# brockpat/JKMP22-Machine-Learning-and-the-Implementable-Efficient-Frontier-Replication

Measured on AMD Instinct MI355X. Metric: PFML hp×window solves/sec (whole node); full grid-search wall-clock, S&P500, higher is better.
Workload: dtype fp64; 1 GPU; global_batch=42824, seq_len=710, parallelism=dp1, dist_backend=none, device=AMD Radeon Graphics, outputs_finite=True, includes_s4_inputs=False, ridge_solve_dtype=fp64 (lambda = 0 / rank-deficient systems: bf16 cannot carry them, SURVEY 7.4), hip_graph=True

## Files before the change

### jkmp22-machine-learning-and-the-implementable-efficient-frontier-replication_amd/csrc/ridge_band.hip

```cpp
#include "common.h"
#include "ridge_desc.h"
#include <cstdlib>
#include <type_traits>

namespace {

constexpr int BB = 16;
constexpr int LS = BB + 1;
constexpr int BMP = 512;
constexpr int BNMAX = BMP + BB;
constexpr int NTR = 512;
constexpr int NWR = NTR / 64;
constexpr int TBR = 4;
constexpr int NTB = 512;
constexpr int NWB = NTB / 64;
constexpr int LC = 16;

__host__ __device__ __forceinline__ int band_npad(int n) { return (n + BB - 1) & ~(BB - 1); }

struct BandWork {
  double *A, *LB, *z, *T, *Yt, *Lf, *F;
  __device__ BandWork(double* w, int n, int L) {
    const int np = (n + BB - 1) / BB;
    const int npad = band_npad(n);
// ... 874 lines not shown
  auto stage_rows = [&](int r0s, int buf) {
    for (int e = threadIdx.x; e < BB * LS; e += NTS) {
      const int r = r0s + e / LS, s = e % LS;
      LBs[buf][e / LS][s] = (r < n) ? LB[(int64_t)r * LS + s] : (s == BB ? 1.0 : 0.0);
    }
  };
  static_assert(BB * LS <= 2 * NTS, "two staged doubles per thread");
  double st[2];
  auto load_rows = [&](int r0s) {
#pragma unroll
    for (int h = 0; h < 2; ++h) {
      const int e = threadIdx.x + h * NTS;
      const int r = r0s + e / LS, s = e % LS;
      st[h] = (e < BB * LS && r < n) ? LB[(int64_t)r * LS + s] : (s == BB ? 1.0 : 0.0);
    }
  };
  auto store_rows = [&](int buf) {
#pragma unroll
    for (int h = 0; h < 2; ++h) {
      const int e = threadIdx.x + h * NTS;
      if (e < BB * LS) LBs[buf][e / LS][e % LS] = st[h];
    }
  };
#pragma unroll
  for (int k = 0; k < 2 * BB; ++k)
    w[k] = (k <= p && p < n) ? LB[(int64_t)p * LS + BB - p + k] + (k == p ? lam : 0.0)
                             : (k == p ? 1.0 : 0.0);
  double zr = (p < n) ? z[p] : 0.0;
  stage_rows(BB, 0);
  double znx = (p + BB < n) ? z[p + BB] : 0.0;
  bool ok = true;
  __syncthreads();

  __builtin_amdgcn_s_waitcnt(0x0F70);
  auto fwd_block = [&](int j0, auto CHECK) {
    constexpr bool chk = decltype(CHECK)::value;
    const int sb = (j0 >> 4) & 1;
    const double lam_in = (j0 + BB + p < n) ? lam : 0.0;
    load_rows(j0 + 2 * BB);
    const double znx2 = (j0 + 2 * BB + p < n) ? z[j0 + 2 * BB + p] : 0.0;
    double myinv = 0.0, myy = 0.0;
    static_for<0, 16>([&](auto U) {
      constexpr int u = decltype(U)::value;
      const int j = j0 + u;
      const bool pl = (p == u);
      double piv = row_bcast<u>(w[u]);
      const double zpiv = row_bcast<u>(zr);
      lds_row_issue<u>(w, lbs_base + (unsigned)(sb * BB * LS + u * LS) * 8u, piv);
      ok = ok && (piv > 0.0);
      double inv = rsqrt1_f64(piv);
      lds_row_wait<u>(w, inv);
      const double yj = zpiv * inv;
      if (pl) {
        w[u + BB] += lam_in;
        zr = znx;
        myinv = inv;
        myy = yj;
      }
      const double lval = w[u] * inv;
      if (!chk || j < n) Lrow[(int64_t)j * BB + (pl ? BB - 1 : ((p - u) & 15) - 1)] = lval;
      zr -= lval * yj;
      static_for<1, LS>([&](auto K) {
        constexpr int k = decltype(K)::value;
        fnmac_bcast<(u + k) & 15, k == 1>(w[u + k], lval, lval);
      });
    });
    if (!chk || j0 + p < n) {
      Linv[j0 + p] = myinv;
      yl[j0 + p] = myy;
    }
#pragma unroll
    for (int s = 0; s < BB; ++s) w[s] = w[s + BB];
    znx = znx2;
    store_rows(sb ^ 1);
    __syncthreads();
  };
  for (int j0 = 0; j0 < npad - 16; j0 += 16) fwd_block(j0, std::false_type{});
  fwd_block(npad - 16, std::true_type{});
  __syncthreads();
  const long long t_mid = (long long)__builtin_amdgcn_s_memtime();
  struct Half {
    double pl[8], iv[8], yv[8];
  };
  auto load_half = [&](int jb, auto S0, auto CHECK, Half& h) {
    constexpr int s0 = decltype(S0)::value;
    static_for<0, 8>([&](auto V) {
      constexpr int v = decltype(V)::value;
      constexpr int u = 15 - s0 - v;
      const int j = jb - s0 - v;
      const int i = (p - u) & 15;
      if constexpr (decltype(CHECK)::value) {
        const bool in = j < n;
        h.pl[v] = in ? Lrow[(int64_t)j * BB + (i == 0 ? BB - 1 : i - 1)] : 0.0;
        h.iv[v] = in ? Linv[j] : 1.0;
        h.yv[v] = in ? yl[j] : 0.0;
      } else {
        const int jc = max(j, 0);
        h.pl[v] = Lrow[(int64_t)jc * BB + (i == 0 ? BB - 1 : i - 1)];
        h.iv[v] = Linv[jc];
        h.yv[v] = yl[jc];
      }
    });
  };
  double xr = 0.0, x1 = 0.0, x2 = 0.0;
  double Pq[2] = {0.0, 0.0}, L1q[2] = {0.0, 0.0}, L2q[2] = {0.0, 0.0};
  auto prep = [&](auto UP, double pl) {
    constexpr int up = decltype(UP)::value & 15;
    const int i = (p - up) & 15;
    const double pm = (i == 1 || i == 2) ? 0.0 : pl;
    Pq[0] = Pq[1];
    L1q[0] = L1q[1];
    L2q[0] = L2q[1];
    Pq[1] = row16_sum(pm * xr);
    L1q[1] = row_bcast<(up + 1) & 15>(pl);
    L2q[1] = row_bcast<(up + 2) & 15>(pl);
  };
  auto step = [&](double yv, double iv) {
    const double t = fma(-L2q[0], x2, yv - Pq[0]);
    const double xj = fma(-L1q[0], x1, t) * iv;
    x2 = x1;
    x1 = xj;
    return xj;
  };
  auto store_half = [&](int jb, int s0) {
    const int j = jb - (15 - p);
    if (lv && j < n && 15 - p >= s0 && 15 - p < s0 + 8) yl[j] = ok ? xr : __builtin_nan("");
  };
  using I0 = std::integral_constant<int, 0>;
  using I8 = std::integral_constant<int, 8>;
  Half A, B;
  load_half(npad - 1, I0{}, std::true_type{}, A);
  {
    Pq[1] = 0.0;
    L1q[1] = row_bcast<0>(A.pl[0]);
    L2q[1] = row_bcast<1>(A.pl[0]);
    Pq[0] = Pq[1]; L1q[0] = L1q[1]; L2q[0] = L2q[1];
    Pq[1] = 0.0;
    L1q[1] = row_bcast<15>(A.pl[1]);
    L2q[1] = row_bcast<0>(A.pl[1]);
  }
  auto block = [&](int jb, auto FIRST) {
    load_half(jb, I8{}, FIRST, B);
    static_for<0, 8>([&](auto V) {
      constexpr int v = decltype(V)::value;
      constexpr int u = 15 - v;
      const double xj = step(A.yv[v], A.iv[v]);
      if constexpr (v + 2 < 8) prep(std::integral_constant<int, u - 2>{}, A.pl[v + 2]);
      else prep(std::integral_constant<int, u - 2>{}, B.pl[v - 6]);
      xr = (p == u) ? xj : xr;
    });
    store_half(jb, 0);
    load_half(jb - 16, I0{}, std::false_type{}, A);
    static_for<0, 8>([&](auto V) {
      constexpr int v = decltype(V)::value;
      constexpr int u = 7 - v;
      const double xj = step(B.yv[v], B.iv[v]);
      if constexpr (v + 2 < 8) prep(std::integral_constant<int, u - 2 + 16>{}, B.pl[v + 2]);
      else prep(std::integral_constant<int, u - 2 + 16>{}, A.pl[v - 6]);
      xr = (p == u) ? xj : xr;
    });
    store_half(jb, 8);
  };
  block(npad - 1, std::true_type{});
  for (int jb = npad - 17; jb >= 0; jb -= 16) block(jb, std::false_type{});
  if (tim != nullptr && blockIdx.x == 0 && threadIdx.x == 0) {
    const long long t_end = (long long)__builtin_amdgcn_s_memtime();
    tim[(int64_t)ncells * 8 + 0] = t_mid - t_start;
    tim[(int64_t)ncells * 8 + 1] = t_end - t_mid;
  }
}

constexpr int LR = BB + 1;
constexpr int UW = 2 * BB + 1;
constexpr int LU_WG = 128;

__global__ __launch_bounds__(256) void band_lu_flag_kernel(const RidgeCellDesc* __restrict__ cells,
                                                           int ncells, int L,
                                                           double* __restrict__ work,
                                                           int* __restrict__ list,
                                                           int* __restrict__ count, int cap) {
  const int e = blockIdx.x * blockDim.x + threadIdx.x;
  if (e >= ncells * L) return;
  const int c = e / L, l = e % L;
  const RidgeCellDesc cd = cells[c];
  const BandWork bw(work + cd.work, cd.n, L);
  const double y0 = bw.Yt[(int64_t)l * cd.n];
  if (y0 != y0) {
    const int slot = atomicAdd(count, 1);
    if (slot < cap) list[slot] = e;
  }
}

__global__ __launch_bounds__(64) void ridge_band_lu_kernel(
    const RidgeCellDesc* __restrict__ cells, const double* __restrict__ lvec, int L,
    double* __restrict__ work, const int* __restrict__ list, const int* __restrict__ count,
    int cap) {
  __shared__ double Us[BNMAX][UW];
  __shared__ double ys[BNMAX];
  __shared__ double W[LR][UW];
  __shared__ double Z[LR];
  const int total = min(*count, cap);
  const int lane = threadIdx.x;
  for (int q = blockIdx.x; q < total; q += gridDim.x) {
    const int e = list[q];
    const RidgeCellDesc cd = cells[e / L];
    const int l = e % L, n = cd.n;
    BandWork bw(work + cd.work, n, L);
    const double lam = lvec[l];
    const double* __restrict__ LB = bw.LB;
    auto band = [&](int r, int c) -> double {
      if (r >= n || c >= n || c < 0 || abs(r - c) > BB) return 0.0;
      const int hi = max(r, c), lo = min(r, c);
      return LB[(int64_t)hi * LS + lo - hi + BB] + (r == c ? lam : 0.0);
    };
    for (int x = lane; x < LR * UW; x += 64) W[x / UW][x % UW] = band(x / UW, x % UW);
    if (lane < LR) Z[lane] = lane < n ? bw.z[lane] : 0.0;
    __syncthreads();
    auto fetch = [&](int k, double& ev, double& zv) {
      const int r = k + LR, c = k + 1 + lane;
      const int hi = max(r, c), lo = min(r, c);
      ev = LB[(int64_t)min(hi, n - 1) * LS + max(0, min(BB, lo - hi + BB))];
      zv = bw.z[min(r, n - 1)];
    };
    auto step = [&](int k, double& ev, double& zv) -> bool {
      const int ks = k % LR, kc = k % UW;
      double a = (lane < LR && k + lane < n) ? fabs(W[(k + lane) % LR][kc]) : -1.0;
      int ia = lane;
#pragma unroll
      for (int off = 16; off > 0; off >>= 1) {
        const double oa = __shfl_xor(a, off, 32);
        const int oi = __shfl_xor(ia, off, 32);
        if (oa > a || (oa == a && oi < ia)) { a = oa; ia = oi; }
      }
      const int ip = __shfl(ia, 0);
      if (ip != 0) {
        const int ps = (k + ip) % LR;
        if (lane < UW) {
          const double t0 = W[ks][lane];
          W[ks][lane] = W[ps][lane];
          W[ps][lane] = t0;
        }
        if (lane == 0) {
          const double t0 = Z[ks];
          Z[ks] = Z[ps];
          Z[ps] = t0;
        }
      }
      __syncthreads();
      const double piv = W[ks][kc];
      if (piv == 0.0 || piv != piv) return false;
      const double rp = 1.0 / piv;
      const double zk = Z[ks];
      if (lane < UW) Us[k][lane] = W[ks][(k + lane) % UW];
      if (lane == 0) ys[k] = zk;
      const int c = 1 + (lane & 31);
      const double uc = W[ks][(k + c) % UW];
      double zm = 0.0;
      if (lane < BB && k + 1 + lane < n) zm = W[(k + 1 + lane) % LR][kc] * rp;
#pragma unroll
      for (int t = 0; t < BB / 2; ++t) {
        const int i = 1 + (lane >> 5) + 2 * t;
        if (k + i < n) {
          const int rs = (k + i) % LR;
          const double m = W[rs][kc] * rp;
          W[rs][(k + c) % UW] -= m * uc;
        }
      }
      if (lane < BB && k + 1 + lane < n) Z[(k + 1 + lane) % LR] -= zm * zk;
      __syncthreads();
      const int r = k + LR, col = k + 1 + lane;
      if (lane < UW)
        W[ks][col % UW] = (r < n && col < n) ? ev + (r == col ? lam : 0.0) : 0.0;
      if (lane < BB) W[(k + 1 + lane) % LR][kc] = 0.0;
      if (lane == 0) Z[ks] = r < n ? zv : 0.0;
      fetch(k + 2, ev, zv);
      __syncthreads();
      return true;
    };
    double eA, zA, eB, zB;
    fetch(0, eA, zA);
    fetch(1, eB, zB);
    bool singular = false;
    for (int k = 0; k < n; k += 2) {
      if (!step(k, eA, zA)) { singular = true; break; }
      if (k + 1 < n && !step(k + 1, eB, zB)) { singular = true; break; }
    }
    if (!singular) {
      for (int k = n - 1; k >= 0; --k) {
        double s = (lane >= 1 && lane < UW && k + lane < n) ? Us[k][lane] * ys[k + lane] : 0.0;
#pragma unroll
        for (int off = 32; off > 0; off >>= 1) s += __shfl_xor(s, off, 64);
        if (lane == 0) ys[k] = (ys[k] - s) / Us[k][0];
        __syncthreads();
      }
      double* __restrict__ yl = bw.Yt + (int64_t)l * n;
      for (int j = lane; j < n; j += 64) yl[j] = ys[j];
    }
    __syncthreads();
  }
}

constexpr int NBW = (BNMAX / 16 + NWB - 1) / NWB;

template <int NWT, int NBT>
__global__ __launch_bounds__(NWT * 64) void ridge_band_backtransform_kernel(
    const RidgeCellDesc* __restrict__ cells, int cell0, int ncells, int L, double* __restrict__ work,
    double* __restrict__ beta_out, int64_t ldo, const unsigned* __restrict__ syncw) {
  __shared__ double red[2][NWT][BB * BB];
  __shared__ double Vw[NWT][NBT][BB][LS];
  const int nch = (L + LC - 1) / LC;
  if ((int)blockIdx.x >= ncells * nch) return;
  const int cell = cell0 + (int)blockIdx.x / nch, ch = blockIdx.x % nch;
  const RidgeCellDesc cd = cells[cell];
  const int n = cd.n;
  const int lane = threadIdx.x & 63;
  const int wid = __builtin_amdgcn_readfirstlane(threadIdx.x >> 6);
  const int c16 = lane & 15, g4 = lane >> 4;
  BandWork bw(work + cd.work, n, L);
  const double* __restrict__ A = bw.A;
  const int l0 = ch * LC;
  const bool lok = c16 < min(LC, L - l0);
  const int nb = (n + 15) >> 4;
  const double* __restrict__ yc = bw.Yt + (int64_t)(l0 + (lok ? c16 : 0)) * n;
  {
    const int lc = min(LC, L - l0), pad = (int)(ldo - n);
    double* __restrict__ o = beta_out + cd.out + (int64_t)l0 * ldo + n;
    for (int e = threadIdx.x; e < lc * pad; e += NWT * 64) o[(int64_t)(e / pad) * ldo + e % pad] = 0.0;
  }
  const bool failed = syncw != nullptr && syncw[(int64_t)cell * COOP_SYNC + 1] != 0u;
  double4_t Y[NBT];
#pragma unroll
  for (int q = 0; q < NBT; ++q)
#pragma unroll
    for (int r = 0; r < 4; ++r) {
      const int i = 16 * (wid + NWT * q) + g4 + 4 * r;
      Y[q][r] = (lok && i < n) ? (failed ? __builtin_nan("") : yc[i]) : 0.0;
    }
  const int lda = band_npad(n);
  double vn[NBT][4], tn[4];
  auto fetch = [&](int p) {
    const int k0 = p * BB, r0 = k0 + BB, m = n - r0;
    const double* Ap = A + (int64_t)r0 * lda + k0;
#pragma unroll
    for (int q = 0; q < NBT; ++q) {
      const int b = wid + NWT * q;
#pragma unroll
      for (int r = 0; r < 4; ++r) {
        const int i = 16 * b - r0 + 4 * r + g4;
        const int ic = min(max(i, 0), m - 1);
        vn[q][r] = Ap[(int64_t)ic * lda + c16];
      }
    }
    const double* Tp = bw.T + (int64_t)p * BB * BB;
#pragma unroll
    for (int r = 0; r < 4; ++r) tn[r] = Tp[c16 * BB + 4 * r + g4];
  };
  const int np = (n - 1) / BB;
  if (np > 0) fetch(np - 1);
  for (int p = np - 1; p >= 0; --p) {
    double (*rp)[BB * BB] = red[p & 1];
    double va[NBT][4], tv[4];
    {
      const int m = n - (p * BB + BB);
#pragma unroll
      for (int q = 0; q < NBT; ++q) {
        const int b = wid + NWT * q;
        const bool live = b > p && b < nb;
#pragma unroll
        for (int r = 0; r < 4; ++r) {
          const int i = 16 * (b - p - 1) + 4 * r + g4;
          va[q][r] = (live && i < m && i >= c16) ? (i == c16 ? 1.0 : vn[q][r]) : 0.0;
        }
      }
    }
#pragma unroll
    for (int r = 0; r < 4; ++r) tv[r] = tn[r];
    if (p > 0) fetch(p - 1);
    double4_t Pp[2] = {{0.0, 0.0, 0.0, 0.0}, {0.0, 0.0, 0.0, 0.0}};
#pragma unroll
    for (int q = 0; q < NBT; ++q) {
      const int b = wid + NWT * q;
      if (b > p && b < nb) {
#pragma unroll
        for (int r = 0; r < 4; ++r) {
          Vw[wid][q][4 * r + g4][c16] = va[q][r];
          Pp[r & 1] = mfma_f64_16x16x4(va[q][r], Y[q][r], Pp[r & 1]);
        }
      }
    }
#pragma unroll
    for (int r = 0; r < 4; ++r) rp[wid][(g4 + 4 * r) * BB + c16] = Pp[0][r] + Pp[1][r];
    __syncthreads();
    double4_t Mm = {0.0, 0.0, 0.0, 0.0};
#pragma unroll
    for (int r = 0; r < 4; ++r) {
      double pv = 0.0;
#pragma unroll
      for (int w = 0; w < NWT; ++w) pv += rp[w][(4 * r + g4) * BB + c16];
      Mm = mfma_f64_16x16x4(tv[r], pv, Mm);
    }
#pragma unroll
    for (int q = 0; q < NBT; ++q) {
      const int b = wid + NWT * q;
      if (b > p && b < nb) {
        double4_t acc = {0.0, 0.0, 0.0, 0.0};
#pragma unroll
        for (int r = 0; r < 4; ++r) acc = mfma_f64_16x16x4(Vw[wid][q][c16][4 * r + g4], Mm[r], acc);
        Y[q] -= acc;
      }
    }
  }
  if (lok) {
    double* __restrict__ out = beta_out + cd.out + (int64_t)(l0 + c16) * ldo;
#pragma unroll
    for (int q = 0; q < NBT; ++q)
#pragma unroll
      for (int r = 0; r < 4; ++r) {
        const int i = 16 * (wid + NWT * q) + g4 + 4 * r;
        if (i < n) out[i] = Y[q][r];
      }
  }
}

}

extern "C" int64_t pfml_ridge_band_work_doubles(int n, int L) {
  const int64_t np = (n + BB - 1) / BB;
  const int64_t npad = band_npad(n);
  const int64_t coop = 2LL * npad * BB + BB * BB + (int64_t)(BNMAX / BB) * (BB * BB + BB);
  return npad * npad + (int64_t)n * LS + n + np * BB * BB + (int64_t)L * n + 15 +
         (int64_t)L * n * LS + coop;
}

extern "C" int pfml_ridge_band_nmax() { return BNMAX; }

namespace {
__global__ __launch_bounds__(NTR) void band_qr_bench_kernel(const double* __restrict__ P, int m,
                                                            int reps,
                                                            double* __restrict__ Aout,
                                                            double* __restrict__ Vout,
                                                            double* __restrict__ Tout,
                                                            long long* __restrict__ cyc) {
  __shared__ double Vs[BMP][LS];
  __shared__ double Gs[BB][LS];
  __shared__ double red[NWR][BB * BB];
  __shared__ double Ts[BB][LS];
  __shared__ double taus[BB];
  const int t = threadIdx.x;
  const int lda = m + BB;
  const double* Pb = P + (int64_t)blockIdx.x * m * BB;
  double* Ab = Aout + (int64_t)blockIdx.x * lda * lda;
  long long acc[8] = {0, 0, 0, 0, 0, 0, 0, 0};
  for (int rep = 0; rep < reps; ++rep) {
    for (int e = t; e < BMP * BB; e += NTR) {
      const int i = e / BB, c = e % BB;
      Vs[i][c] = (i < m) ? Pb[e] : 0.0;
    }
    __syncthreads();
    long long tk[6] = {0, 0, 0, 0, 0, 0};
    const long long t0 = (long long)__builtin_amdgcn_s_memtime();
    band_panel_hh(Ab, lda, 0, BB, m, Vs, Gs, &red[0][0], Ts, taus,
                  Tout + (int64_t)blockIdx.x * BB * BB, t == 0 ? tk : nullptr, Vs);
    __syncthreads();
    const long long t1 = (long long)__builtin_amdgcn_s_memtime();
    acc[0] += t1 - t0;
    acc[1] += tk[0] - t0;
    acc[2] += tk[1] - tk[0];
    acc[3] += t1 - tk[1];
    acc[4] += tk[2];
    acc[5] += tk[3];
    acc[6] += tk[4];
  }
  for (int e = t; e < m * BB; e += NTR) Vout[(int64_t)blockIdx.x * m * BB + e] = Vs[e / BB][e % BB];
  if (t == 0)
    for (int q = 0; q < 8; ++q) cyc[(int64_t)blockIdx.x * 8 + q] = acc[q] / (reps > 0 ? reps : 1);
}
}

extern "C" hipError_t pfml_band_qr_bench(const double* P, int m, int nblocks, int reps,
                                         double* Aout, double* Vout, double* Tout,
                                         long long* cyc, hipStream_t st) {
  if (m < 1 || m > BMP) return hipErrorInvalidValue;
  hipLaunchKernelGGL(band_qr_bench_kernel, dim3(nblocks), dim3(NTR), 0, st, P, m, reps, Aout,
                     Vout, Tout, cyc);
  return hipGetLastError();
}

static int g_coop_solo = 1;
extern "C" void pfml_coop_set_solo(int on) { g_coop_solo = on ? 1 : 0; }

extern "C" void pfml_coop_set_spin_max(unsigned n) { g_coop_spin_max = n ? n : COOP_SPIN_MAX; }

namespace {
template <int NWT, int NBT>
void bt_one(const RidgeCellDesc* cd, int c0, int nc, int L, double* work, double* beta_out,
            int64_t ldo, const unsigned* syncw, hipStream_t st) {
  const int nch = (L + LC - 1) / LC;
  hipLaunchKernelGGL((ridge_band_backtransform_kernel<NWT, NBT>), dim3(nc * nch), dim3(NWT * 64),
                     0, st, cd, c0, nc, L, work, beta_out, ldo, syncw);
}

int bt_class(int n) { return n <= 96 ? 0 : (n <= 192 ? 1 : (n <= 320 ? 2 : 3)); }

void ridge_band_bt_launch(const RidgeCellDesc* cd, const int* n_host, int ncells, int L,
                          double* work, double* beta_out, int64_t ldo, const unsigned* syncw,
                          hipStream_t st) {
  if (n_host == nullptr) {
    bt_one<NWB, NBW>(cd, 0, ncells, L, work, beta_out, ldo, syncw, st);
    return;
  }
  int c0 = 0;
  while (c0 < ncells) {
    const int k = bt_class(n_host[c0]);
    int c1 = c0 + 1;
    while (c1 < ncells && bt_class(n_host[c1]) == k) ++c1;
    switch (k) {
      case 0: bt_one<2, 3>(cd, c0, c1 - c0, L, work, beta_out, ldo, syncw, st); break;
      case 1: bt_one<4, 3>(cd, c0, c1 - c0, L, work, beta_out, ldo, syncw, st); break;
      case 2: bt_one<4, 5>(cd, c0, c1 - c0, L, work, beta_out, ldo, syncw, st); break;
      default: bt_one<NWB, NBW>(cd, c0, c1 - c0, L, work, beta_out, ldo, syncw, st); break;
    }
    c0 = c1;
  }
}
}

extern "C" hipError_t pfml_ridge_band_launch(const double* SD, int64_t ldS, const double* Sr,
                                             const void* cells, int ncells, const double* lvec,
                                             int L, double* work, double* beta_out, int64_t ldo,
                                             long long* tim, int* lu_list, int* lu_count,
                                             int lu_cap, const int* wgmap, int nwg,
                                             unsigned* syncw, const int* n_host,
                                             hipStream_t st) {
  const RidgeCellDesc* cd = static_cast<const RidgeCellDesc*>(cells);
  if (wgmap == nullptr || syncw == nullptr || nwg <= 0)
    return hipErrorInvalidValue;
  hipError_t e = hipMemsetAsync(syncw, 0, (size_t)ncells * COOP_SYNC * sizeof(unsigned), st);
  if (e != hipSuccess) return e;
  const bool solo = g_coop_solo != 0 && nwg == ncells;
#define COOP_LAUNCH(TIMED, SOLO)                                                            \
  hipLaunchKernelGGL((band_coop_kernel<TIMED, SOLO>), dim3(nwg), dim3(NTR), 0, st, SD, ldS, Sr, \
                     cd, L, work, wgmap, syncw, tim, g_coop_spin_max)
  if (tim != nullptr) {
    if (solo) COOP_LAUNCH(true, true);
    else COOP_LAUNCH(true, false);
  } else {
    if (solo) COOP_LAUNCH(false, true);
    else COOP_LAUNCH(false, false);
  }
#undef COOP_LAUNCH
  hipLaunchKernelGGL(ridge_band_solve_kernel, dim3(ncells * ((L + 15) / 16)), dim3(NTS), 0, st,
                     cd, lvec, L, work,
                     tim != nullptr ? tim + (int64_t)ncells * 8 : tim, ncells,
                     lu_count);
  if (lu_count != nullptr) {
    hipLaunchKernelGGL(band_lu_flag_kernel, dim3((ncells * L + 255) / 256), dim3(256), 0, st, cd,
                       ncells, L, work, lu_list, lu_count, lu_cap);
    hipLaunchKernelGGL(ridge_band_lu_kernel, dim3(LU_WG), dim3(64), 0, st, cd, lvec, L, work,
                       lu_list, lu_count, lu_cap);
  }
  const int nch = (L + LC - 1) / LC;
  ridge_band_bt_launch(cd, n_host, ncells, L, work, beta_out, ldo, syncw, st);
  return hipGetLastError();
}
```

Measured before the change: 9.353 million solves/s.

## Cut backtransform LDS and registers to raise occupancy, per-q prefetch

Shrinks the per-wave shared Vw buffer from NBT tiles to a single 16x16 tile reused per block, with wave-level barriers guarding the transpose through LDS. It drops the separate va/vn/tn register arrays, masks the V tile in place, loads T each step, and interleaves the next panel's fetch per q after each update. It also adds a min-waves-per-SIMD launch bound, a sched_barrier, 32-bit offset addressing and an opaque index to cut register pressure. The goal is higher occupancy and lower LDS use, at the cost of less prefetch distance and extra wave barriers.

```diff
diff --git a/jkmp22-machine-learning-and-the-implementable-efficient-frontier-replication_amd/csrc/ridge_band.hip b/jkmp22-machine-learning-and-the-implementable-efficient-frontier-replication_amd/csrc/ridge_band.hip
--- a/jkmp22-machine-learning-and-the-implementable-efficient-frontier-replication_amd/csrc/ridge_band.hip
+++ b/jkmp22-machine-learning-and-the-implementable-efficient-frontier-replication_amd/csrc/ridge_band.hip
@@ -1200,12 +1200,14 @@
 
 constexpr int NBW = (BNMAX / 16 + NWB - 1) / NWB;
 
+constexpr int BT_WPS = 4;
+
 template <int NWT, int NBT>
-__global__ __launch_bounds__(NWT * 64) void ridge_band_backtransform_kernel(
+__global__ __launch_bounds__(NWT * 64, BT_WPS) void ridge_band_backtransform_kernel(
     const RidgeCellDesc* __restrict__ cells, int cell0, int ncells, int L, double* __restrict__ work,
     double* __restrict__ beta_out, int64_t ldo, const unsigned* __restrict__ syncw) {
   __shared__ double red[2][NWT][BB * BB];
-  __shared__ double Vw[NWT][NBT][BB][LS];
+  __shared__ double Vw[NWT][BB][LS];
   const int nch = (L + LC - 1) / LC;
   if ((int)blockIdx.x >= ncells * nch) return;
   const int cell = cell0 + (int)blockIdx.x / nch, ch = blockIdx.x % nch;
@@ -1235,45 +1237,33 @@
       Y[q][r] = (lok && i < n) ? (failed ? __builtin_nan("") : yc[i]) : 0.0;
     }
   const int lda = band_npad(n);
-  double vn[NBT][4], tn[4];
-  auto fetch = [&](int p) {
+  double vv[NBT][4];
+  auto fetch = [&](int p, int q) {
     const int k0 = p * BB, r0 = k0 + BB, m = n - r0;
     const double* Ap = A + (int64_t)r0 * lda + k0;
-#pragma unroll
-    for (int q = 0; q < NBT; ++q) {
-      const int b = wid + NWT * q;
-#pragma unroll
-      for (int r = 0; r < 4; ++r) {
-        const int i = 16 * b - r0 + 4 * r + g4;
-        const int ic = min(max(i, 0), m - 1);
-        vn[q][r] = Ap[(int64_t)ic * lda + c16];
-      }
-    }
-    const double* Tp = bw.T + (int64_t)p * BB * BB;
-#pragma unroll
-    for (int r = 0; r < 4; ++r) tn[r] = Tp[c16 * BB + 4 * r + g4];
+    const int b = wid + NWT * q;
+#pragma unroll
+    for (int r = 0; r < 4; ++r) {
+      const int i = 16 * b - r0 + 4 * r + g4;
+      const int ic = min(max(i, 0), m - 1);
+      vv[q][r] = *reinterpret_cast<const double*>(reinterpret_cast<const char*>(Ap) +
+                                                  (unsigned)((ic * lda + c16) * 8));
+    }
   };
   const int np = (n - 1) / BB;
-  if (np > 0) fetch(np - 1);
+  if (np > 0) {
+#pragma unroll
+    for (int q = 0; q < NBT; ++q) fetch(np - 1, q);
+  }
   for (int p = np - 1; p >= 0; --p) {
     double (*rp)[BB * BB] = red[p & 1];
-    double va[NBT][4], tv[4];
+    double tv[4];
     {
-      const int m = n - (p * BB + BB);
-#pragma unroll
-      for (int q = 0; q < NBT; ++q) {
-        const int b = wid + NWT * q;
-        const bool live = b > p && b < nb;
-#pragma unroll
-        for (int r = 0; r < 4; ++r) {
-          const int i = 16 * (b - p - 1) + 4 * r + g4;
-          va[q][r] = (live && i < m && i >= c16) ? (i == c16 ? 1.0 : vn[q][r]) : 0.0;
-        }
-      }
-    }
-#pragma unroll
-    for (int r = 0; r < 4; ++r) tv[r] = tn[r];
-    if (p > 0) fetch(p - 1);
+      const double* Tp = bw.T + (int64_t)p * BB * BB;
+#pragma unroll
+      for (int r = 0; r < 4; ++r) tv[r] = Tp[c16 * BB + 4 * r + g4];
+    }
+    const int m = n - (p * BB + BB);
     double4_t Pp[2] = {{0.0, 0.0, 0.0, 0.0}, {0.0, 0.0, 0.0, 0.0}};
 #pragma unroll
     for (int q = 0; q < NBT; ++q) {
@@ -1281,8 +1271,9 @@
       if (b > p && b < nb) {
 #pragma unroll
         for (int r = 0; r < 4; ++r) {
-          Vw[wid][q][4 * r + g4][c16] = va[q][r];
-          Pp[r & 1] = mfma_f64_16x16x4(va[q][r], Y[q][r], Pp[r & 1]);
+          const int i = 16 * (b - p - 1) + 4 * r + g4;
+          vv[q][r] = (i < m && i >= c16) ? (i == c16 ? 1.0 : vv[q][r]) : 0.0;
+          Pp[r & 1] = mfma_f64_16x16x4(vv[q][r], Y[q][r], Pp[r & 1]);
         }
       }
     }
@@ -1296,25 +1287,40 @@
 #pragma unroll
       for (int w = 0; w < NWT; ++w) pv += rp[w][(4 * r + g4) * BB + c16];
       Mm = mfma_f64_16x16x4(tv[r], pv, Mm);
+      __builtin_amdgcn_sched_barrier(0);
     }
 #pragma unroll
     for (int q = 0; q < NBT; ++q) {
       const int b = wid + NWT * q;
       if (b > p && b < nb) {
+#pragma unroll
+        for (int r = 0; r < 4; ++r) Vw[wid][4 * r + g4][c16] = vv[q][r];
+        __builtin_amdgcn_fence(__ATOMIC_RELEASE, "wavefront");
+        __builtin_amdgcn_wave_barrier();
+        __builtin_amdgcn_fence(__ATOMIC_ACQUIRE, "wavefront");
+        double vt[4];
+#pragma unroll
+        for (int r = 0; r < 4; ++r) vt[r] = Vw[wid][c16][4 * r + g4];
+        __builtin_amdgcn_fence(__ATOMIC_RELEASE, "wavefront");
+        __builtin_amdgcn_wave_barrier();
+        __builtin_amdgcn_fence(__ATOMIC_ACQUIRE, "wavefront");
         double4_t acc = {0.0, 0.0, 0.0, 0.0};
 #pragma unroll
-        for (int r = 0; r < 4; ++r) acc = mfma_f64_16x16x4(Vw[wid][q][c16][4 * r + g4], Mm[r], acc);
+        for (int r = 0; r < 4; ++r) acc = mfma_f64_16x16x4(vt[r], Mm[r], acc);
         Y[q] -= acc;
       }
+      if (p > 0) fetch(p - 1, q);
     }
   }
   if (lok) {
     double* __restrict__ out = beta_out + cd.out + (int64_t)(l0 + c16) * ldo;
+    int i0 = 16 * wid + g4;
+    asm volatile("" : "+v"(i0));
 #pragma unroll
     for (int q = 0; q < NBT; ++q)
 #pragma unroll
       for (int r = 0; r < 4; ++r) {
-        const int i = 16 * (wid + NWT * q) + g4 + 4 * r;
+        const int i = i0 + 16 * NWT * q + 4 * r;
         if (i < n) out[i] = Y[q][r];
       }
   }
```

Result: faster. 9.546 million solves/s (median of 6 runs) (+2.1%).
